# vwxyzjn/cleanrl

Measured on NVIDIA H100. Metric: env steps/sec (SPS) PPO Breakout num_envs=1024, higher is better.
Workload: dtype bf16

## Files before the change

cleanrl_b200/csrc/net_tc.cu:

```cuda
#include <cuda.h>
#include <algorithm>
#include "tc_base.cuh"
#include "tc_conv_win.cuh"
#include "tc_conv1_u8.cuh"
#include "tc_gemm_tma.cuh"
#include "tc_wgrad_win.cuh"
#include "tc_reduce.cuh"
#include "tc_aux.cuh"
#include "tc_heads.cuh"
#include "tc_heads_wide.cuh"
#include "tc_lstm.cuh"

namespace b200rl {

struct NatureLayout {
    int A;
    int64_t c1w, c1b, c2w, c2b, c3w, c3b, fcw, fcb, hw, hb, total;
    int64_t w1f, w2f, w2dg, w3f, w3dg, wfcf, wfcdg, w1l, w1sc, packed_total;
    bool wide; int G; int64_t whf, whdg, hbp;
    int64_t wih, whh, bih, bhh, whhp;
    explicit NatureLayout(int A_) : A(A_), wih(-1), whh(-1), bih(-1), bhh(-1), whhp(-1) {
        int64_t o = 0;
        c1w = o; o += 32 * 4 * 8 * 8;  c1b = o; o += 32;
        c2w = o; o += 64 * 32 * 4 * 4; c2b = o; o += 64;
        c3w = o; o += 64 * 64 * 3 * 3; c3b = o; o += 64;
        fcw = o; o += 512 * 3136;      fcb = o; o += 512;
        hw = o;  o += (int64_t)(A + 1) * 512;
        hb = o;  o += A + 1;
        total = o;
        int64_t q = 0;
        w1f = q; q += 32 * 256;
        w2f = q; q += 64 * 512;
        w2dg = q; q += 4 * 32 * 256;
        w3f = q; q += 64 * 576;
        w3dg = q; q += 64 * 576;
        wfcf = q; q += 512 * 3136;
        wfcdg = q; q += 3136 * 512;
        w1l = q; q += 64 * 256 / 2;
        w1sc = q; q += 64 * 2;
        wide = A + 1 > kMaxHeads;
        G = wide ? (int)ceil_div(A + 1, kWideHeadPad) * kWideHeadPad : 0;
        whf = whdg = hbp = 0;
        if (wide) {
            whf = q; q += (int64_t)G * 512;
            whdg = q; q += (int64_t)G * 512;
            hbp = q; q += (int64_t)G * 2;
        }
        packed_total = q;
    }
    struct Lstm {};
    NatureLayout(int A_, Lstm) : A(A_) {
        int64_t o = 0;
        c1w = o; o += 32 * 8 * 8;      c1b = o; o += 32;
        c2w = o; o += 64 * 32 * 4 * 4; c2b = o; o += 64;
        c3w = o; o += 64 * 64 * 3 * 3; c3b = o; o += 64;
        fcw = o; o += 512 * 3136;      fcb = o; o += 512;
// ... 9 lines not shown
        w3f = q; q += 64 * 576;
        w3dg = q; q += 64 * 576;
        wfcf = q; q += 512 * 3136;
        wfcdg = q; q += 3136 * 512;
        w1l = w1sc = -1;
        wide = true; G = 512;
        whf = q; q += 512 * 512;
        whdg = q; q += 512 * 512;
        hbp = q; q += 512 * 2;
        whhp = q; q += 512 * 128;
        packed_total = q;
    }
};

struct NatureActs {
    int64_t x0, act1, act2, act3, hid, dhid, dact3a, dact3b, dact2a, dact2b, dact1, m1, m2, m3, m4, total;
    explicit NatureActs(int64_t n, bool with_x0 = true) {
        int64_t o = 0;
        x0 = o; if (with_x0) o += n * 28224;
        act1 = o; o += n * 12800;
        act2 = o; o += n * 5184;
        act3 = o; o += n * 3136;
        hid = o;  o += n * 512;
        dhid = o; o += n * 512;
        dact3a = o; o += n * 5184;
        dact3b = o; o += n * 7744;
        dact2a = o; o += n * 6400;
        dact2b = o; o += n * 7744;
        dact1 = o; o += n * 14112;
        auto pad8 = [](int64_t v) { return (v + 7) & ~int64_t(7); };
        m1 = o; o += pad8(n * 100 * 4 * 2);
        m2 = o; o += pad8(n * 81 * 2 * 2);
        m3 = o; o += pad8(n * 49 * 2 * 2);
        m4 = o; o += pad8(n * 16 * 2);
        total = o;
    }
};

static void gemm_rowmajor(KGemmParams& p, const bf16* x, int64_t n, int nchunks) {
    memset(&p, 0, sizeof(p));
    p.scale = 1.f;
    p.A = x; p.M = n; p.nchunks = nchunks;
}


static void win_defaults(WinParams& p) { memset(&p, 0, sizeof(p)); p.scale = 1.f; }
static int round8(int v) { return (v + 7) & ~7; }
static void win_conv1(WinParams& p, const bf16* x0, const int64_t* rows, int64_t n) {
    p.A = x0; p.rows = rows; p.n = (int)n; p.G = 441; p.Wp = 21; p.M = n * 441;
    p.tpi_shift = 2;
    p.n_images = rows ? (int64_t)1 << 24 : n;
    p.ntaps = 4; p.shift[0] = 0; p.shift[1] = 1; p.shift[2] = 21; p.shift[3] = 22; p.WR = round8(128 + 22);
}
static void win_conv2(WinParams& p, const bf16* act1, int64_t n) {
    p.A = act1; p.n = (int)n; p.G = 100; p.Wp = 10; p.M = n * 100;
    p.ntaps = 4; p.shift[0] = 0; p.shift[1] = 1; p.shift[2] = 10; p.shift[3] = 11; p.WR = round8(128 + 11);
}
static void win_conv3(WinParams& p, const bf16* act2, int64_t n) {
    p.A = act2; p.n = (int)n; p.G = 81; p.Wp = 9; p.M = n * 81;
    p.ntaps = 9; for (int ky = 0; ky < 3; ++ky) for (int kx = 0; kx < 3; ++kx) p.shift[ky * 3 + kx] = ky * 9 + kx;
    p.WR = round8(128 + 20);
}
static void wgw_defaults(WGradWinParams& w) { memset(&w, 0, sizeof(w)); }

static const int kC1Ctas = 264, kC2Ctas = 132, kC3Ctas = 132;
static WPlan conv1_wgrad_plan(int64_t n, bool u8) {
    return u8 ? wgrad_plan(n * 512, kC2Ctas, 512) : wgrad_plan(n * 512, kC1Ctas, 128);
}
static WPlan conv2_wgrad_plan(int64_t n) { return wgrad_plan(n * 100, kC2Ctas, 128); }
static WPlan conv3_wgrad_plan(int64_t n) { return wgrad_plan(n * 81, kC3Ctas, 128); }

static size_t wgrad_win_bytes(int splits, int nslots) { return (size_t)splits * nslots * 64 * 64 * sizeof(float); }
static size_t wgrad_win_bias_bytes(int splits) { return (size_t)splits * 64 * sizeof(float); }
static int launch_wgrad_win(const WGradWinParams& p, int ctas, cudaStream_t s, const char* what) {
    const size_t smem = (size_t)kWgradWinStages * ((size_t)p.WRX * 128 * p.cpr + 128 * 128) + 4096 + 1024;
    static SmemAttrCache attr;
    if (int rc0 = attr.ensure(tc_wgrad_win, smem, what)) return rc0;
    CUtensorMap tmX, tmY;
    memset(&tmX, 0, sizeof(tmX)); memset(&tmY, 0, sizeof(tmY));
    const int use_tma = p.tpi_shift ? 0 : 1;
    if (p.rows_per_cta % 128 != 0) return fail(B200RL_ERR_INVALID_ARGUMENT, "%s: rows per CTA must be a multiple of 128", what);
    if (ctas < 1 || (int64_t)(ctas - 1) * p.rows_per_cta >= p.M)
        return fail(B200RL_ERR_INVALID_ARGUMENT, "%s: every row split must own at least one row", what);
    int rc;
    if (use_tma) {
        if (p.rows || p.ldy != 64 || p.ncolsY != 64)
            return fail(B200RL_ERR_INVALID_ARGUMENT, "%s: linear-grid mode needs contiguous rows and 64-channel dY", what);
        if ((rc = make_tmap_2d(&tmX, p.X, p.M, (int64_t)p.cpr * 64, p.WRX, what))) return rc;
        if ((rc = make_tmap_2d(&tmY, p.Y, p.M, 64, 128, what))) return rc;
    } else {
        if ((128 << p.tpi_shift) < p.G) return fail(B200RL_ERR_INVALID_ARGUMENT, "%s: steps per image too small", what);
        if ((rc = make_tmap_3d(&tmX, p.X, p.n_images, p.G, (int64_t)p.cpr * 64, p.WRX, what))) return rc;
    }
    const dim3 grid((unsigned)ceil_div(p.nslots / 2, kWgradWinTilesPerCta), ctas);
    tc_wgrad_win<<<grid, kWgradWinThreads, smem, s>>>(tmX, tmY, p, use_tma);
    return check_launch(what);
}

}

using namespace b200rl;

namespace b200rl {
static bool head_ok(int A) { return A >= 1 && A < kMaxWideHeads; }
static size_t wide_dhead_bytes(int64_t n, const NatureLayout& L) { return ((size_t)n * L.G * 2 + 255) & ~(size_t)255; }
static size_t wide_small_bytes(int64_t n, const NatureLayout& L, int A1) {
    return wide_dhead_bytes(n, L) + colsum_f32_ws(n, A1);
}

static int trunk_fwd(const NatureLayout& L, const NatureActs& Q, const float* params, const bf16* P, bf16* act, int64_t n,
                     cudaStream_t s) {
    int rc;
    KGemmParams p;
    WinParams wp;
    win_defaults(wp); win_conv2(wp, act + Q.act1, n);
    wp.Bw = P + L.w2f; wp.N = 64; wp.vH = 9; wp.vW = 9; wp.out_mode = WOUT_DENSE; wp.out = act + Q.act2;
    wp.bias = params + L.c2b; wp.relu = 1; wp.mask_out = reinterpret_cast<uint32_t*>(act + Q.m2);
    { ProfScope ps(s, "conv2_fwd", 2.0 * n * 81 * 64 * 512, (double)n * ((12800 + 5184) * 2 + 648));
      if (n <= 8192) { if ((rc = launch_conv_win_t<64, 2, 6, 4>(wp, s, "naturecnn/conv2"))) return rc; }
      else if ((rc = launch_conv_win_t<128, 2, 2, 4>(wp, s, "naturecnn/conv2"))) return rc; }
    win_defaults(wp); win_conv3(wp, act + Q.act2, n);
    wp.Bw = P + L.w3f; wp.N = 64; wp.vH = 7; wp.vW = 7; wp.out_mode = WOUT_DENSE; wp.out = act + Q.act3;
    wp.bias = params + L.c3b; wp.relu = 1; wp.mask_out = reinterpret_cast<uint32_t*>(act + Q.m3);
    { ProfScope ps(s, "conv3_fwd", 2.0 * n * 49 * 64 * 576, (double)n * ((5184 + 3136) * 2 + 392));
      if (n <= 8192) { if ((rc = launch_conv_win_t<64, 1, 8, 9>(wp, s, "naturecnn/conv3"))) return rc; }
      else if ((rc = launch_conv_win_t<128, 1, 4, 9>(wp, s, "naturecnn/conv3"))) return rc; }
    gemm_rowmajor(p, act + Q.act3, n, 49);
    p.Bw = P + L.wfcf; p.N = 512; p.out = act + Q.hid; p.ldo = 512; p.bias = params + L.fcb; p.relu = 1;
    p.mask_out = reinterpret_cast<uint32_t*>(act + Q.m4);
    { ProfScope ps(s, "fc_fwd", 2.0 * n * 512 * 3136, (double)n * (3136 + 512) * 2 + 512.0 * 3136 * 2);
      if (n <= 8192) { if ((rc = launch_gemm_tma<64, 6>(p, s, "naturecnn/fc"))) return rc; }
      else if ((rc = launch_gemm_tma<128, 3>(p, s, "naturecnn/fc"))) return rc; }
    return B200RL_OK;
}

static int trunk_bwd(const NatureLayout& L, const NatureActs& Q, const bf16* P, bf16* act, float* grads, int64_t n,
                     float* wsbig, float* wssmall, void* tail_ready_event, bool dact1_fused, cudaStream_t s) {
    int rc;
    KGemmParams p;
    {
        int splits;
        { ProfScope ps(s, "fc_wgrad", 2.0 * n * 512 * 3136, (double)n * (3136 + 512) * 2 + 512.0 * 3136 * 4);
          if ((splits = launch_wgrad_tma(act + Q.dhid, 512, act + Q.act3, 3136, n, wsbig, s, "naturecnn/fc_wgrad")) < 0) return splits; }
        { ProfScope ps(s, "wgrad_fold_bias", 0, 0);
          note_launches(1); tc_fold_fc<<<(unsigned)ceil_div((int64_t)512 * 3136, 256), 256, 0, s>>>(wsbig, splits, 512, 13 * 256, 512, 3136, 64, 49, 1.f, grads + L.fcw);
          if ((rc = colsum(act + Q.dhid, n, 512, 512, wssmall, grads + L.fcb, s))) return rc; }
        if (tail_ready_event) {
            cudaError_t e = cudaEventRecord(reinterpret_cast<cudaEvent_t>(tail_ready_event), s);
            if (e != cudaSuccess) return fail(B200RL_ERR_CUDA, "naturecnn_backward: cudaEventRecord: %s", cudaGetErrorString(e));
        }
        gemm_rowmajor(p, act + Q.dhid, n, 8);
        p.Bw = P + L.wfcdg; p.N = 3136; p.out = act + Q.dact3a; p.out2 = act + Q.dact3b; p.dual_dact3 = 1;
        p.ldo = 3136; p.mask_bits = reinterpret_cast<const uint32_t*>(act + Q.m3);
        { ProfScope ps(s, "fc_dgrad", 2.0 * n * 512 * 3136, (double)n * ((3136 + 512) * 2 + 392) + 512.0 * 3136 * 2);
          if ((rc = launch_gemm_tma<128, 3>(p, s, "naturecnn/fc_dgrad"))) return rc; }
    }
    WGradWinParams gw;
    WinParams wp;
    FoldWin fw;
    {
        wgw_defaults(gw);
        gw.X = act + Q.act2; gw.M = n * 81; gw.n = (int)n; gw.G = 81; gw.cpr = 1; gw.nslots = 10; gw.WRX = round8(128 + 20);
        for (int t = 0; t < 9; ++t) gw.shift[t] = (t / 3) * 9 + (t % 3);
        const int st[10] = {0, 1, 2, 3, 4, 5, 6, 7, 7, 8};
        for (int k = 0; k < 10; ++k) { gw.slot_tap[k] = st[k]; gw.slot_cc[k] = 0; }
        gw.Y = act + Q.dact3a; gw.ldy = 64; gw.ncolsY = 64;
        const WPlan pl = conv3_wgrad_plan(n);
        gw.rows_per_cta = pl.rows_per_cta; gw.ws = wsbig; gw.wsb = wssmall;
        { ProfScope ps(s, "conv3_wgrad", 2.0 * n * 49 * 64 * 576, (double)n * (5184 + 5184) * 2);
          if ((rc = launch_wgrad_win(gw, pl.splits, s, "naturecnn/conv3_wgrad"))) return rc; }
        memset(&fw, 0, sizeof(fw));
        fw.layer = 3; fw.S = pl.splits; fw.nslots = 10; fw.Cout = 64; fw.scale = 1.f; fw.bscale = 1.f;
        for (int k = 0; k < 10; ++k) { fw.slot_tap[k] = st[k]; fw.slot_skip[k] = (k == 8); }
        { ProfScope ps(s, "wgrad_fold_bias", 0, 0);
          fw.wsb = wssmall; fw.db = grads + L.c3b;
          tc_fold_win<<<(unsigned)ceil_div(640 * 64 + 64, 32), 256, 0, s>>>(wsbig, fw, grads + L.c3w);
          if ((rc = check_launch("naturecnn/conv3_fold"))) return rc; }
        win_defaults(wp);
        wp.A = act + Q.dact3b; wp.n = (int)n; wp.G = 121; wp.Wp = 11; wp.M = n * 121; wp.ntaps = 9;
// ... 462 lines not shown
```

cleanrl_b200/csrc/tc_conv_win.cuh:

```cuda
#pragma once
#include "tc_base.cuh"

namespace b200rl {
using namespace tc;

enum { WOUT_DENSE = 0, WOUT_S2D2 = 1, WOUT_DACT2 = 2, WOUT_DACT1 = 3 };
struct WinParams {
    const bf16* A;
    const int64_t* rows;
    int64_t M;
    int n, G, Wp;
    int tpi_shift;
    int64_t n_images;
    int ntaps;
    int shift[16];
    int WR;
    const bf16* Bw;
    int N;
    int vH, vW;
    int out_mode;
    bf16* out;
    bf16* out2;
    const uint32_t* mask_bits;
    uint32_t* mask_out;
// ... 219 lines not shown
}

template <int BN, int CPR, int STAGES, int NTAPS>
static int launch_conv_win(const WinParams& p, cudaStream_t s, const char* what) {
    if (p.ntaps != NTAPS) return fail(B200RL_ERR_INVALID_ARGUMENT, "%s: %d taps, kernel instance has %d", what, p.ntaps, NTAPS);
    if (p.out_mode != WOUT_S2D2 && p.out_mode != WOUT_DACT1)
        return fail(B200RL_ERR_INVALID_ARGUMENT, "%s: dense and conv3 data-gradient outputs run on tc_conv_win_t", what);
    if (p.out_mode == WOUT_DACT1 && (BN != 128 || p.N != 128))
        return fail(B200RL_ERR_INVALID_ARGUMENT, "%s: the conv2 data gradient stores 4 groups of 32 channels per cell", what);
    const size_t smem = (size_t)p.ntaps * CPR * BN * 128 + (size_t)STAGES * p.WR * 128 * CPR + conv_win_acc_bytes<BN>() + 1024;
    static SmemAttrCache attr;
    if (int rc = attr.ensure(tc_conv_win<BN, CPR, STAGES, NTAPS>, smem, what)) return rc;
    if ((int64_t)p.G * p.Wp >= 65536 || p.G < 1 || p.N % 32 != 0)
        return fail(B200RL_ERR_INVALID_ARGUMENT, "%s: grid %d x width %d outside the epilogue's multiply-shift range, or N %% 32 != 0", what, p.G, p.Wp);
    if (p.rows && !p.tpi_shift) return fail(B200RL_ERR_INVALID_ARGUMENT, "%s: the image gather needs image-aligned tiling", what);
    if (p.tpi_shift && (128 << p.tpi_shift) < p.G) return fail(B200RL_ERR_INVALID_ARGUMENT, "%s: tiles per image too small", what);
    const int total = p.tpi_shift ? (int)((int64_t)p.n << p.tpi_shift) : (int)ceil_div(p.M, 128);
    int grid = num_sms();
    if (grid > total) grid = total;
    CUtensorMap tmA, tmW;
    memset(&tmA, 0, sizeof(tmA));
    memset(&tmW, 0, sizeof(tmW));
    int rc;
    if (p.tpi_shift) rc = make_tmap_3d(&tmA, p.A, p.n_images, p.G, (int64_t)CPR * 64, p.WR, what);
    else rc = make_tmap_2d(&tmA, p.A, p.M, (int64_t)CPR * 64, p.WR, what);
    if (rc) return rc;
    if ((rc = make_tmap_2d(&tmW, p.Bw, p.N, (int64_t)NTAPS * CPR * 64, BN, what))) return rc;
    tc_conv_win<BN, CPR, STAGES, NTAPS><<<grid, kConvWinThreads, smem, s>>>(tmA, tmW, p, total);
    return check_launch(what);
}

constexpr int kConvWinTThreads = 384;
constexpr int kConvWinTLds = 64 + 4;
template <int BP>
__host__ __device__ constexpr size_t conv_win_t_stage_bytes() { return (size_t)2 * BP * kConvWinTLds * sizeof(float); }

template <int R>
__device__ __forceinline__ void stage_acc_transposed(float* st, int wg_tid, const float (&d)[R]) {
    const int co = ((wg_tid >> 5) << 4) + ((wg_tid & 31) >> 2), pos = (wg_tid & 3) * 2;
#pragma unroll
    for (int j = 0; j < R / 4; ++j) {
        float* p0 = st + (8 * j + pos) * kConvWinTLds + co;
        p0[0] = d[4 * j];
        p0[kConvWinTLds] = d[4 * j + 1];
        p0[8] = d[4 * j + 2];
        p0[kConvWinTLds + 8] = d[4 * j + 3];
    }
}

template <int BP, int CPR, int STAGES, int NTAPS>
__global__ void __launch_bounds__(kConvWinTThreads, 1) tc_conv_win_t(const __grid_constant__ CUtensorMap tmA,
                                                                     const __grid_constant__ CUtensorMap tmW, const WinParams p,
                                                                     int total_tiles) {
    static_assert(BP == 64 || BP % 128 == 0, "the epilogue's 128 threads per warpgroup cover whole position rows");
    static_assert(STAGES % 2 == 0, "each consumer warpgroup owns every other stage");
    constexpr int TPP = BP >= 128 ? 1 : 2;
    constexpr int PPR = 128 / TPP;
    constexpr int RPT = BP >= 128 ? BP / 128 : 1;
    constexpr int A_CHUNK = 64 * 128;
    constexpr int LDS = kConvWinTLds;
    extern __shared__ uint8_t smem_raw[];
    __shared__ uint64_t full_bar[STAGES], empty_bar[STAGES], w_bar;
    uint8_t* smem = smem_raw + ((1024u - (smem_u32(smem_raw) & 1023u)) & 1023u);
    const int tid = threadIdx.x, warp = tid >> 5;
    const int nchunks = NTAPS * CPR;
    const int IMG = p.WR * 128;
    const int STAGE_BYTES = IMG * CPR;
    uint8_t* sW = smem;
    uint8_t* sRing = smem + (size_t)nchunks * A_CHUNK;
    float* sAcc = reinterpret_cast<float*>(sRing + (size_t)STAGES * STAGE_BYTES);

    if (tid == 0) {
        for (int s = 0; s < STAGES; ++s) { mbar_init(&full_bar[s], 1); mbar_init(&empty_bar[s], 4); }
        mbar_init(&w_bar, 1);
        fence_barrier_init();
        tma_prefetch_desc(&tmA);
        tma_prefetch_desc(&tmW);
    }
    __syncthreads();
    const int tile_begin = (int)(((int64_t)total_tiles * blockIdx.x) / gridDim.x);
    const int tile_end = (int)(((int64_t)total_tiles * (blockIdx.x + 1)) / gridDim.x);

    if (warp == 0) {
        if (tid == 0) {
            uint32_t q = 0;
            for (int tile = tile_begin; tile < tile_end; ++tile, ++q) {
                const uint32_t s = q % STAGES;
                if (q >= (uint32_t)STAGES) mbar_wait(&empty_bar[s], ((q / STAGES) - 1) & 1);
                const uint32_t dst = smem_u32(sRing + (size_t)s * STAGE_BYTES);
                mbar_arrive_expect_tx(&full_bar[s], (uint32_t)STAGE_BYTES);
#pragma unroll
                for (int c = 0; c < CPR; ++c) tma_load_2d(dst + c * IMG, &tmA, c * 64, tile * BP, &full_bar[s]);
                if (q == 0) {
                    mbar_arrive_expect_tx(&w_bar, (uint32_t)(nchunks * A_CHUNK));
                    for (int j = 0; j < nchunks; ++j) tma_load_2d(smem_u32(sW + (size_t)j * A_CHUNK), &tmW, j * 64, 0, &w_bar);
                }
            }
        }
    } else if (warp >= 4) {
        const int wg = (warp - 4) >> 2, wt = tid & 127;
        float* st = sAcc + wg * BP * LDS;
        const uint32_t w_base = smem_u32(sW);
        const uint32_t mW = (65536u + (uint32_t)p.Wp - 1u) / (uint32_t)p.Wp;
        constexpr int NW = 2;
        const int pw = wt % PPR, gq = wt / PPR;
        float d[BP / 2];
#pragma unroll
        for (int e = 0; e < BP / 2; ++e) d[e] = 0.f;
        if (tile_begin + wg < tile_end) mbar_wait(&w_bar, 0);
        for (int tile = tile_begin + wg; tile < tile_end; tile += 2) {
            const uint32_t q = (uint32_t)(tile - tile_begin), s = q % STAGES;
            mbar_wait(&full_bar[s], (q / STAGES) & 1);
            wgmma_fence();
            const uint32_t win = smem_u32(sRing + (size_t)s * STAGE_BYTES);
#pragma unroll
            for (int t = 0; t < NTAPS; ++t) {
#pragma unroll
                for (int c = 0; c < CPR; ++c) {
                    const uint64_t b = desc_kmajor(win + (uint32_t)(c * IMG) + (uint32_t)p.shift[t] * 128u);
                    const uint64_t a = desc_kmajor(w_base + (uint32_t)((t * CPR + c) * A_CHUNK));
#pragma unroll
                    for (int kk = 0; kk < 4; ++kk)
                        WgmmaBf16<BP, 0, 0>::mma(d, a + 2 * kk, b + 2 * kk, (t | c | kk) != 0 ? 1u : 0u);
                }
            }
            wgmma_commit();
            bool valid[RPT];
            int64_t o1[RPT], o2[RPT], ob[RPT];
            uint32_t mb[RPT][NW];
#pragma unroll
            for (int rr = 0; rr < RPT; ++rr) {
                const int64_t r = (int64_t)tile * BP + rr * PPR + pw;
                const int i = (int)(r / p.G);
                const int rem = (int)(r - (int64_t)i * p.G);
                const int Y = (int)(((uint32_t)rem * mW) >> 16), X = rem - Y * p.Wp;
                valid[rr] = r < p.M && (Y < p.vH) && (X < p.vW);
                o2[rr] = 0;
                if (p.out_mode == WOUT_DENSE) {
                    const int64_t orow = ((int64_t)i * p.vH + Y) * p.vW + X;
                    o1[rr] = orow * p.N; ob[rr] = orow * (p.N >> 5);
                } else {
                    o1[rr] = ((int64_t)i * 100 + Y * 10 + X) * 64;
                    o2[rr] = ((int64_t)i * 121 + (Y + 1) * 11 + (X + 1)) * 64;
                    ob[rr] = ((int64_t)i * 81 + Y * 9 + X) * 2;
                }
                mb[rr][0] = mb[rr][1] = 0xFFFFFFFFu;
                if (p.mask_bits != nullptr && valid[rr]) {
                    const uint2 t = __ldg(reinterpret_cast<const uint2*>(p.mask_bits + ob[rr]));
                    mb[rr][0] = t.x; mb[rr][1] = t.y;
                }
            }
            wgmma_wait<0>();
            wgmma_fence_operands(d);
            if ((tid & 31) == 0) mbar_arrive(&empty_bar[s]);
            named_bar(1 + wg, 128);
            stage_acc_transposed(st, wt, d);
            named_bar(1 + wg, 128);
#pragma unroll
            for (int rr = 0; rr < RPT; ++rr) {
                float* srow = st + (rr * PPR + pw) * LDS;
#pragma unroll
                for (int g = 0; g < NW; ++g) {
                    if (TPP == 2 && g != gq) continue;
                    if (TPP == 1 && (!valid[rr] || g * 32 >= p.N)) continue;
                    uint32_t v[32];
#pragma unroll
                    for (int e = 0; e < 8; ++e) {
                        const float4 f = *reinterpret_cast<const float4*>(srow + g * 32 + 4 * e);
                        v[4 * e] = __float_as_uint(f.x); v[4 * e + 1] = __float_as_uint(f.y);
                        v[4 * e + 2] = __float_as_uint(f.z); v[4 * e + 3] = __float_as_uint(f.w);
                    }
                    if (TPP == 2) {
                        named_bar(1 + wg, 128);
                        if (!valid[rr] || g * 32 >= p.N) continue;
                    }
                    if (p.bias) {
                        const float4* bp = reinterpret_cast<const float4*>(p.bias + g * 32);
#pragma unroll
                        for (int e = 0; e < 8; ++e) {
                            const float4 bv = __ldg(bp + e);
                            v[4 * e] = __float_as_uint(fmaf(__uint_as_float(v[4 * e]), p.scale, bv.x));
                            v[4 * e + 1] = __float_as_uint(fmaf(__uint_as_float(v[4 * e + 1]), p.scale, bv.y));
                            v[4 * e + 2] = __float_as_uint(fmaf(__uint_as_float(v[4 * e + 2]), p.scale, bv.z));
                            v[4 * e + 3] = __float_as_uint(fmaf(__uint_as_float(v[4 * e + 3]), p.scale, bv.w));
                        }
                    } else {
#pragma unroll
                        for (int e = 0; e < 32; ++e) v[e] = __float_as_uint(__uint_as_float(v[e]) * p.scale);
                    }
                    if (p.relu) {
                        uint32_t bits = 0u;
#pragma unroll
                        for (int e = 0; e < 32; ++e) bits |= (__uint_as_float(v[e]) > 0.f ? 1u : 0u) << e;
                        if (p.mask_out) p.mask_out[ob[rr] + g] = bits;
                    }
                    if (p.mask_bits) {
#pragma unroll
                        for (int e = 0; e < 32; ++e) if (!((mb[rr][g] >> e) & 1u)) v[e] = 0u;
                    }
                    int4 w[4];
                    if (p.relu) {
#pragma unroll
                        for (int e = 0; e < 4; ++e) {
                            w[e].x = (int)pack_bf16x2_relu(__uint_as_float(v[8 * e]), __uint_as_float(v[8 * e + 1]));
                            w[e].y = (int)pack_bf16x2_relu(__uint_as_float(v[8 * e + 2]), __uint_as_float(v[8 * e + 3]));
                            w[e].z = (int)pack_bf16x2_relu(__uint_as_float(v[8 * e + 4]), __uint_as_float(v[8 * e + 5]));
                            w[e].w = (int)pack_bf16x2_relu(__uint_as_float(v[8 * e + 6]), __uint_as_float(v[8 * e + 7]));
                        }
                    } else {
#pragma unroll
                        for (int e = 0; e < 4; ++e) {
                            w[e].x = (int)pack_bf16x2(__uint_as_float(v[8 * e]), __uint_as_float(v[8 * e + 1]));
                            w[e].y = (int)pack_bf16x2(__uint_as_float(v[8 * e + 2]), __uint_as_float(v[8 * e + 3]));
                            w[e].z = (int)pack_bf16x2(__uint_as_float(v[8 * e + 4]), __uint_as_float(v[8 * e + 5]));
                            w[e].w = (int)pack_bf16x2(__uint_as_float(v[8 * e + 6]), __uint_as_float(v[8 * e + 7]));
                        }
                    }
                    int4* brow = reinterpret_cast<int4*>(srow) + 4 * g;
#pragma unroll
                    for (int e = 0; e < 4; ++e) brow[e] = w[e];
                }
                if (gq == 0) *reinterpret_cast<longlong2*>(srow + 64) = make_longlong2(valid[rr] ? o1[rr] : -1, o2[rr]);
            }
            named_bar(1 + wg, 128);
#pragma unroll
            for (int m = 0; m < BP / 16; ++m) {
                const int k = m * 128 + wt, part = k & 7;
                const float* srow = st + (k >> 3) * LDS;
                const longlong2 off = *reinterpret_cast<const longlong2*>(srow + 64);
                if (off.x < 0) continue;
                const int4 val = reinterpret_cast<const int4*>(srow)[part];
                *reinterpret_cast<int4*>(p.out + off.x + part * 8) = val;
                if (p.out_mode == WOUT_DACT2) *reinterpret_cast<int4*>(p.out2 + off.y + part * 8) = val;
            }
        }
    }
}

template <int BP, int CPR, int STAGES, int NTAPS>
static int launch_conv_win_t(WinParams p, cudaStream_t s, const char* what) {
    if (p.ntaps != NTAPS) return fail(B200RL_ERR_INVALID_ARGUMENT, "%s: %d taps, kernel instance has %d", what, p.ntaps, NTAPS);
    if (p.N != 64) return fail(B200RL_ERR_INVALID_ARGUMENT, "%s: N = %d, the kernel computes 64 output channels", what, p.N);
    if ((int64_t)p.G * p.Wp >= 65536 || p.G < 1)
        return fail(B200RL_ERR_INVALID_ARGUMENT, "%s: grid %d x width %d outside the epilogue's multiply-shift range", what, p.G, p.Wp);
    if (p.rows || p.tpi_shift) return fail(B200RL_ERR_INVALID_ARGUMENT, "%s: the channel-major kernel walks a contiguous linear grid", what);
    if (p.out_mode != WOUT_DENSE && p.out_mode != WOUT_DACT2)
        return fail(B200RL_ERR_INVALID_ARGUMENT, "%s: only bf16 dense and conv3 data-gradient outputs in this kernel", what);
    int maxs = 0;
    for (int t = 0; t < NTAPS; ++t) maxs = p.shift[t] > maxs ? p.shift[t] : maxs;
    p.WR = (BP + maxs + 7) & ~7;
    if (p.WR > 256) return fail(B200RL_ERR_INVALID_ARGUMENT, "%s: window of %d rows exceeds a TMA box", what, p.WR);
    const size_t smem = (size_t)NTAPS * CPR * 64 * 128 + (size_t)STAGES * p.WR * 128 * CPR + conv_win_t_stage_bytes<BP>() + 1024;
    static SmemAttrCache attr;
    if (int rc = attr.ensure(tc_conv_win_t<BP, CPR, STAGES, NTAPS>, smem, what)) return rc;
    const int total = (int)ceil_div(p.M, BP);
    int grid = num_sms();
    if (grid > total) grid = total;
    CUtensorMap tmA, tmW;
    memset(&tmA, 0, sizeof(tmA));
    memset(&tmW, 0, sizeof(tmW));
    if (int rc = make_tmap_2d(&tmA, p.A, p.M, (int64_t)CPR * 64, p.WR, what)) return rc;
    if (int rc = make_tmap_2d(&tmW, p.Bw, 64, (int64_t)NTAPS * CPR * 64, 64, what)) return rc;
    tc_conv_win_t<BP, CPR, STAGES, NTAPS><<<grid, kConvWinTThreads, smem, s>>>(tmA, tmW, p, total);
    return check_launch(what);
}

}
```

cleanrl_b200/csrc/tc_wgmma.cuh:

```cuda
#pragma once
#include <cstdint>

namespace b200rl { namespace tc {

__device__ __forceinline__ void wgmma_fence() { asm volatile("wgmma.fence.sync.aligned;" ::: "memory"); }
__device__ __forceinline__ void wgmma_commit() { asm volatile("wgmma.commit_group.sync.aligned;" ::: "memory"); }
template <int N>
__device__ __forceinline__ void wgmma_wait() { asm volatile("wgmma.wait_group.sync.aligned %0;" ::"n"(N) : "memory"); }
template <class T, int R>
__device__ __forceinline__ void wgmma_fence_operands(T (&d)[R]) {
#pragma unroll
    for (int i = 0; i < R; ++i) asm volatile("" : "+r"(reinterpret_cast<uint32_t&>(d[i]))::"memory");
}

template <int N, int TA, int TB> struct WgmmaBf16;
template <int TA, int TB> struct WgmmaBf16<32, TA, TB> {
    __device__ __forceinline__ static void mma(float (&d)[16], uint64_t adesc, uint64_t bdesc, uint32_t accumulate) {
        asm volatile(
            "{\n\t.reg .pred p;\n\tsetp.ne.b32 p, %18, 0;\n\t"
            "wgmma.mma_async.sync.aligned.m64n32k16.f32.bf16.bf16 {"
            "%0, %1, %2, %3, %4, %5, %6, %7, %8, %9, %10, %11, %12, %13, %14, %15"
            "}, %16, %17, p, 1, 1, %19, %20;\n\t}\n"
            : "+f"(d[0]), "+f"(d[1]), "+f"(d[2]), "+f"(d[3]), "+f"(d[4]), "+f"(d[5]), "+f"(d[6]), "+f"(d[7]),
              "+f"(d[8]), "+f"(d[9]), "+f"(d[10]), "+f"(d[11]), "+f"(d[12]), "+f"(d[13]), "+f"(d[14]), "+f"(d[15])
            : "l"(adesc), "l"(bdesc), "r"(accumulate), "n"(TA), "n"(TB));
    }
};
template <int TA, int TB> struct WgmmaBf16<64, TA, TB> {
    __device__ __forceinline__ static void mma(float (&d)[32], uint64_t adesc, uint64_t bdesc, uint32_t accumulate) {
        asm volatile(
            "{\n\t.reg .pred p;\n\tsetp.ne.b32 p, %34, 0;\n\t"
            "wgmma.mma_async.sync.aligned.m64n64k16.f32.bf16.bf16 {"
            "%0, %1, %2, %3, %4, %5, %6, %7, %8, %9, %10, %11, %12, %13, %14, %15, "
            "%16, %17, %18, %19, %20, %21, %22, %23, %24, %25, %26, %27, %28, %29, %30, %31"
            "}, %32, %33, p, 1, 1, %35, %36;\n\t}\n"
            : "+f"(d[0]), "+f"(d[1]), "+f"(d[2]), "+f"(d[3]), "+f"(d[4]), "+f"(d[5]), "+f"(d[6]), "+f"(d[7]),
              "+f"(d[8]), "+f"(d[9]), "+f"(d[10]), "+f"(d[11]), "+f"(d[12]), "+f"(d[13]), "+f"(d[14]), "+f"(d[15]),
              "+f"(d[16]), "+f"(d[17]), "+f"(d[18]), "+f"(d[19]), "+f"(d[20]), "+f"(d[21]), "+f"(d[22]), "+f"(d[23]),
              "+f"(d[24]), "+f"(d[25]), "+f"(d[26]), "+f"(d[27]), "+f"(d[28]), "+f"(d[29]), "+f"(d[30]), "+f"(d[31])
            : "l"(adesc), "l"(bdesc), "r"(accumulate), "n"(TA), "n"(TB));
    }
};
template <int TA, int TB> struct WgmmaBf16<128, TA, TB> {
    __device__ __forceinline__ static void mma(float (&d)[64], uint64_t adesc, uint64_t bdesc, uint32_t accumulate) {
        asm volatile(
            "{\n\t.reg .pred p;\n\tsetp.ne.b32 p, %66, 0;\n\t"
            "wgmma.mma_async.sync.aligned.m64n128k16.f32.bf16.bf16 {"
            "%0, %1, %2, %3, %4, %5, %6, %7, %8, %9, %10, %11, %12, %13, %14, %15, "
            "%16, %17, %18, %19, %20, %21, %22, %23, %24, %25, %26, %27, %28, %29, %30, %31, "
            "%32, %33, %34, %35, %36, %37, %38, %39, %40, %41, %42, %43, %44, %45, %46, %47, "
            "%48, %49, %50, %51, %52, %53, %54, %55, %56, %57, %58, %59, %60, %61, %62, %63"
            "}, %64, %65, p, 1, 1, %67, %68;\n\t}\n"
            : "+f"(d[0]), "+f"(d[1]), "+f"(d[2]), "+f"(d[3]), "+f"(d[4]), "+f"(d[5]), "+f"(d[6]), "+f"(d[7]),
              "+f"(d[8]), "+f"(d[9]), "+f"(d[10]), "+f"(d[11]), "+f"(d[12]), "+f"(d[13]), "+f"(d[14]), "+f"(d[15]),
              "+f"(d[16]), "+f"(d[17]), "+f"(d[18]), "+f"(d[19]), "+f"(d[20]), "+f"(d[21]), "+f"(d[22]), "+f"(d[23]),
              "+f"(d[24]), "+f"(d[25]), "+f"(d[26]), "+f"(d[27]), "+f"(d[28]), "+f"(d[29]), "+f"(d[30]), "+f"(d[31]),
              "+f"(d[32]), "+f"(d[33]), "+f"(d[34]), "+f"(d[35]), "+f"(d[36]), "+f"(d[37]), "+f"(d[38]), "+f"(d[39]),
              "+f"(d[40]), "+f"(d[41]), "+f"(d[42]), "+f"(d[43]), "+f"(d[44]), "+f"(d[45]), "+f"(d[46]), "+f"(d[47]),
              "+f"(d[48]), "+f"(d[49]), "+f"(d[50]), "+f"(d[51]), "+f"(d[52]), "+f"(d[53]), "+f"(d[54]), "+f"(d[55]),
              "+f"(d[56]), "+f"(d[57]), "+f"(d[58]), "+f"(d[59]), "+f"(d[60]), "+f"(d[61]), "+f"(d[62]), "+f"(d[63])
            : "l"(adesc), "l"(bdesc), "r"(accumulate), "n"(TA), "n"(TB));
    }
};
template <int TA, int TB> struct WgmmaBf16<256, TA, TB> {
    __device__ __forceinline__ static void mma(float (&d)[128], uint64_t adesc, uint64_t bdesc, uint32_t accumulate) {
        asm volatile(
            "{\n\t.reg .pred p;\n\tsetp.ne.b32 p, %130, 0;\n\t"
            "wgmma.mma_async.sync.aligned.m64n256k16.f32.bf16.bf16 {"
            "%0, %1, %2, %3, %4, %5, %6, %7, %8, %9, %10, %11, %12, %13, %14, %15, "
            "%16, %17, %18, %19, %20, %21, %22, %23, %24, %25, %26, %27, %28, %29, %30, %31, "
            "%32, %33, %34, %35, %36, %37, %38, %39, %40, %41, %42, %43, %44, %45, %46, %47, "
            "%48, %49, %50, %51, %52, %53, %54, %55, %56, %57, %58, %59, %60, %61, %62, %63, "
            "%64, %65, %66, %67, %68, %69, %70, %71, %72, %73, %74, %75, %76, %77, %78, %79, "
            "%80, %81, %82, %83, %84, %85, %86, %87, %88, %89, %90, %91, %92, %93, %94, %95, "
            "%96, %97, %98, %99, %100, %101, %102, %103, %104, %105, %106, %107, %108, %109, %110, %111, "
            "%112, %113, %114, %115, %116, %117, %118, %119, %120, %121, %122, %123, %124, %125, %126, %127"
            "}, %128, %129, p, 1, 1, %131, %132;\n\t}\n"
            : "+f"(d[0]), "+f"(d[1]), "+f"(d[2]), "+f"(d[3]), "+f"(d[4]), "+f"(d[5]), "+f"(d[6]), "+f"(d[7]),
              "+f"(d[8]), "+f"(d[9]), "+f"(d[10]), "+f"(d[11]), "+f"(d[12]), "+f"(d[13]), "+f"(d[14]), "+f"(d[15]),
              "+f"(d[16]), "+f"(d[17]), "+f"(d[18]), "+f"(d[19]), "+f"(d[20]), "+f"(d[21]), "+f"(d[22]), "+f"(d[23]),
              "+f"(d[24]), "+f"(d[25]), "+f"(d[26]), "+f"(d[27]), "+f"(d[28]), "+f"(d[29]), "+f"(d[30]), "+f"(d[31]),
              "+f"(d[32]), "+f"(d[33]), "+f"(d[34]), "+f"(d[35]), "+f"(d[36]), "+f"(d[37]), "+f"(d[38]), "+f"(d[39]),
              "+f"(d[40]), "+f"(d[41]), "+f"(d[42]), "+f"(d[43]), "+f"(d[44]), "+f"(d[45]), "+f"(d[46]), "+f"(d[47]),
              "+f"(d[48]), "+f"(d[49]), "+f"(d[50]), "+f"(d[51]), "+f"(d[52]), "+f"(d[53]), "+f"(d[54]), "+f"(d[55]),
              "+f"(d[56]), "+f"(d[57]), "+f"(d[58]), "+f"(d[59]), "+f"(d[60]), "+f"(d[61]), "+f"(d[62]), "+f"(d[63]),
              "+f"(d[64]), "+f"(d[65]), "+f"(d[66]), "+f"(d[67]), "+f"(d[68]), "+f"(d[69]), "+f"(d[70]), "+f"(d[71]),
              "+f"(d[72]), "+f"(d[73]), "+f"(d[74]), "+f"(d[75]), "+f"(d[76]), "+f"(d[77]), "+f"(d[78]), "+f"(d[79]),
              "+f"(d[80]), "+f"(d[81]), "+f"(d[82]), "+f"(d[83]), "+f"(d[84]), "+f"(d[85]), "+f"(d[86]), "+f"(d[87]),
              "+f"(d[88]), "+f"(d[89]), "+f"(d[90]), "+f"(d[91]), "+f"(d[92]), "+f"(d[93]), "+f"(d[94]), "+f"(d[95]),
              "+f"(d[96]), "+f"(d[97]), "+f"(d[98]), "+f"(d[99]), "+f"(d[100]), "+f"(d[101]), "+f"(d[102]), "+f"(d[103]),
              "+f"(d[104]), "+f"(d[105]), "+f"(d[106]), "+f"(d[107]), "+f"(d[108]), "+f"(d[109]), "+f"(d[110]), "+f"(d[111]),
              "+f"(d[112]), "+f"(d[113]), "+f"(d[114]), "+f"(d[115]), "+f"(d[116]), "+f"(d[117]), "+f"(d[118]), "+f"(d[119]),
// ... 35 lines not shown
```

Baseline: 1.281 million.

## Fuse conv2 and conv3 forward into one persistent per-image kernel

Replaces the separate conv2 and conv3 windowed-conv launches with one persistent kernel that processes a whole image per warpgroup. conv2 output is built in shared memory (bias, ReLU, mask bits) and fed straight into conv3's wgmma, while act2 is still written to global memory for backward. This removes one launch and the global round trip of act2 between the two convs. The cost is a fixed per-image schedule with more synchronisation, padded 96-column conv2 tiles, and a single CTA per SM. The now-unused BP=64 path in the old window-conv kernel is removed.

After: 1.330 million, median of 6. 1.04x the previous value.

```diff
diff --git a/cleanrl_b200/csrc/net_tc.cu b/cleanrl_b200/csrc/net_tc.cu
--- a/cleanrl_b200/csrc/net_tc.cu
+++ b/cleanrl_b200/csrc/net_tc.cu
@@ -2,6 +2,7 @@
 #include <algorithm>
 #include "tc_base.cuh"
 #include "tc_conv_win.cuh"
+#include "tc_conv23.cuh"
 #include "tc_conv1_u8.cuh"
 #include "tc_gemm_tma.cuh"
 #include "tc_wgrad_win.cuh"
@@ -117,15 +118,6 @@
     p.n_images = rows ? (int64_t)1 << 24 : n;
     p.ntaps = 4; p.shift[0] = 0; p.shift[1] = 1; p.shift[2] = 21; p.shift[3] = 22; p.WR = round8(128 + 22);
 }
-static void win_conv2(WinParams& p, const bf16* act1, int64_t n) {
-    p.A = act1; p.n = (int)n; p.G = 100; p.Wp = 10; p.M = n * 100;
-    p.ntaps = 4; p.shift[0] = 0; p.shift[1] = 1; p.shift[2] = 10; p.shift[3] = 11; p.WR = round8(128 + 11);
-}
-static void win_conv3(WinParams& p, const bf16* act2, int64_t n) {
-    p.A = act2; p.n = (int)n; p.G = 81; p.Wp = 9; p.M = n * 81;
-    p.ntaps = 9; for (int ky = 0; ky < 3; ++ky) for (int kx = 0; kx < 3; ++kx) p.shift[ky * 3 + kx] = ky * 9 + kx;
-    p.WR = round8(128 + 20);
-}
 static void wgw_defaults(WGradWinParams& w) { memset(&w, 0, sizeof(w)); }
 
 static const int kC1Ctas = 264, kC2Ctas = 132, kC3Ctas = 132;
@@ -177,19 +169,12 @@
                      cudaStream_t s) {
     int rc;
     KGemmParams p;
-    WinParams wp;
-    win_defaults(wp); win_conv2(wp, act + Q.act1, n);
-    wp.Bw = P + L.w2f; wp.N = 64; wp.vH = 9; wp.vW = 9; wp.out_mode = WOUT_DENSE; wp.out = act + Q.act2;
-    wp.bias = params + L.c2b; wp.relu = 1; wp.mask_out = reinterpret_cast<uint32_t*>(act + Q.m2);
-    { ProfScope ps(s, "conv2_fwd", 2.0 * n * 81 * 64 * 512, (double)n * ((12800 + 5184) * 2 + 648));
-      if (n <= 8192) { if ((rc = launch_conv_win_t<64, 2, 6, 4>(wp, s, "naturecnn/conv2"))) return rc; }
-      else if ((rc = launch_conv_win_t<128, 2, 2, 4>(wp, s, "naturecnn/conv2"))) return rc; }
-    win_defaults(wp); win_conv3(wp, act + Q.act2, n);
-    wp.Bw = P + L.w3f; wp.N = 64; wp.vH = 7; wp.vW = 7; wp.out_mode = WOUT_DENSE; wp.out = act + Q.act3;
-    wp.bias = params + L.c3b; wp.relu = 1; wp.mask_out = reinterpret_cast<uint32_t*>(act + Q.m3);
-    { ProfScope ps(s, "conv3_fwd", 2.0 * n * 49 * 64 * 576, (double)n * ((5184 + 3136) * 2 + 392));
-      if (n <= 8192) { if ((rc = launch_conv_win_t<64, 1, 8, 9>(wp, s, "naturecnn/conv3"))) return rc; }
-      else if ((rc = launch_conv_win_t<128, 1, 4, 9>(wp, s, "naturecnn/conv3"))) return rc; }
+    Conv23Params cp;
+    cp.n = (int)n; cp.b2 = params + L.c2b; cp.b3 = params + L.c3b; cp.act2 = act + Q.act2; cp.act3 = act + Q.act3;
+    cp.m2 = reinterpret_cast<uint32_t*>(act + Q.m2); cp.m3 = reinterpret_cast<uint32_t*>(act + Q.m3);
+    { ProfScope ps(s, "conv23_fwd", 2.0 * n * 81 * 64 * 512 + 2.0 * n * 49 * 64 * 576,
+                   (double)n * (12800 * 2 + 5184 * 2 + 648 + 3136 * 2 + 392));
+      if ((rc = launch_conv23_fwd(act + Q.act1, P + L.w2f, P + L.w3f, cp, s, "naturecnn/conv23"))) return rc; }
     gemm_rowmajor(p, act + Q.act3, n, 49);
     p.Bw = P + L.wfcf; p.N = 512; p.out = act + Q.hid; p.ldo = 512; p.bias = params + L.fcb; p.relu = 1;
     p.mask_out = reinterpret_cast<uint32_t*>(act + Q.m4);
diff --git a/cleanrl_b200/csrc/tc_conv23.cuh b/cleanrl_b200/csrc/tc_conv23.cuh
--- /dev/null
+++ b/cleanrl_b200/csrc/tc_conv23.cuh
@@ -0,0 +1,218 @@
+#pragma once
+#include "tc_conv_win.cuh"
+
+namespace b200rl {
+using namespace tc;
+
+struct Conv23Params {
+    int n;
+    const float* b2;
+    const float* b3;
+    bf16* act2;
+    bf16* act3;
+    uint32_t* m2;
+    uint32_t* m3;
+};
+
+constexpr int kConv23Threads = 384;
+constexpr int kC23WinRows = 112;
+constexpr int kC23Chunk = 64 * 128;
+constexpr int kC23StageBytes = 2 * kC23WinRows * 128;
+constexpr int kC23ImgBytes = 64 * 64 * 4;
+constexpr size_t kC23Smem = (size_t)(8 + 9) * kC23Chunk + 2 * kC23StageBytes + 2 * kC23ImgBytes + 1024;
+static_assert(96 * kConvWinTLds * 4 <= kC23StageBytes, "conv2's fp32 staging fits its window stage");
+static_assert(88 * 128 <= kC23ImgBytes, "the act2 image and its zero tail fit the conv3 staging");
+
+__device__ __forceinline__ uint32_t conv23_group(const float* srow, int g, int sw, const float* bias, int4 (&w)[4]) {
+    float v[32];
+    const float4* bp = reinterpret_cast<const float4*>(bias + g * 32);
+#pragma unroll
+    for (int e = 0; e < 8; ++e) {
+        const float4 f = reinterpret_cast<const float4*>(srow)[(8 * g + e) ^ sw];
+        const float4 bv = __ldg(bp + e);
+        v[4 * e] = fmaf(f.x, 1.f, bv.x); v[4 * e + 1] = fmaf(f.y, 1.f, bv.y);
+        v[4 * e + 2] = fmaf(f.z, 1.f, bv.z); v[4 * e + 3] = fmaf(f.w, 1.f, bv.w);
+    }
+    uint32_t bits = 0u;
+#pragma unroll
+    for (int e = 0; e < 32; ++e) bits |= (v[e] > 0.f ? 1u : 0u) << e;
+#pragma unroll
+    for (int e = 0; e < 4; ++e) {
+        w[e].x = (int)pack_bf16x2_relu(v[8 * e], v[8 * e + 1]);
+        w[e].y = (int)pack_bf16x2_relu(v[8 * e + 2], v[8 * e + 3]);
+        w[e].z = (int)pack_bf16x2_relu(v[8 * e + 4], v[8 * e + 5]);
+        w[e].w = (int)pack_bf16x2_relu(v[8 * e + 6], v[8 * e + 7]);
+    }
+    return bits;
+}
+
+__device__ __forceinline__ void stage_acc_transposed_sw(float* st, int wg_tid, const float (&d)[32]) {
+    const int co = ((wg_tid >> 5) << 4) + ((wg_tid & 31) >> 2), pos = (wg_tid & 3) * 2;
+#pragma unroll
+    for (int j = 0; j < 8; ++j) {
+        const int r0 = 8 * j + pos, r1 = r0 + 1;
+        st[r0 * 64 + (co ^ ((r0 & 7) << 2))] = d[4 * j];
+        st[r1 * 64 + (co ^ ((r1 & 7) << 2))] = d[4 * j + 1];
+        st[r0 * 64 + ((co + 8) ^ ((r0 & 7) << 2))] = d[4 * j + 2];
+        st[r1 * 64 + ((co + 8) ^ ((r1 & 7) << 2))] = d[4 * j + 3];
+    }
+}
+
+__global__ void __launch_bounds__(kConv23Threads, 1) tc_conv23_fwd(const __grid_constant__ CUtensorMap tmA,
+                                                                   const __grid_constant__ CUtensorMap tmW2,
+                                                                   const __grid_constant__ CUtensorMap tmW3, const Conv23Params p) {
+    constexpr int IMG = kC23WinRows * 128;
+    constexpr int LDS = kConvWinTLds;
+    extern __shared__ uint8_t smem_raw[];
+    __shared__ uint64_t full_bar[2], empty_bar[2], w2_bar, w3_bar;
+    uint8_t* smem = smem_raw + ((1024u - (smem_u32(smem_raw) & 1023u)) & 1023u);
+    const int tid = threadIdx.x, warp = tid >> 5;
+    uint8_t* sW2 = smem;
+    uint8_t* sW3 = sW2 + 8 * kC23Chunk;
+    uint8_t* sRing = sW3 + 9 * kC23Chunk;
+    uint8_t* sImg = sRing + 2 * kC23StageBytes;
+
+    if (tid == 0) {
+        for (int s = 0; s < 2; ++s) { mbar_init(&full_bar[s], 1); mbar_init(&empty_bar[s], 4); }
+        mbar_init(&w2_bar, 1);
+        mbar_init(&w3_bar, 1);
+        fence_barrier_init();
+        tma_prefetch_desc(&tmA);
+        tma_prefetch_desc(&tmW2);
+        tma_prefetch_desc(&tmW3);
+    }
+    __syncthreads();
+    const int img_begin = (int)(((int64_t)p.n * blockIdx.x) / gridDim.x);
+    const int img_end = (int)(((int64_t)p.n * (blockIdx.x + 1)) / gridDim.x);
+
+    if (warp == 0) {
+        if (tid == 0) {
+            bool w3_sent = false;
+            uint32_t q = 0;
+            for (int img = img_begin; img < img_end; ++img, ++q) {
+                const uint32_t s = q & 1;
+                if (q >= 2) mbar_wait(&empty_bar[s], ((q >> 1) - 1) & 1);
+                const uint32_t dst = smem_u32(sRing + (size_t)s * kC23StageBytes);
+                mbar_arrive_expect_tx(&full_bar[s], (uint32_t)kC23StageBytes);
+                tma_load_3d(dst, &tmA, 0, 0, img, &full_bar[s]);
+                tma_load_3d(dst + IMG, &tmA, 64, 0, img, &full_bar[s]);
+                if (q == 0) {
+                    mbar_arrive_expect_tx(&w2_bar, (uint32_t)(8 * kC23Chunk));
+                    for (int j = 0; j < 8; ++j) tma_load_2d(smem_u32(sW2 + (size_t)j * kC23Chunk), &tmW2, j * 64, 0, &w2_bar);
+                }
+                if (!w3_sent && (q == 1 || img + 1 == img_end)) {
+                    mbar_arrive_expect_tx(&w3_bar, (uint32_t)(9 * kC23Chunk));
+                    for (int j = 0; j < 9; ++j) tma_load_2d(smem_u32(sW3 + (size_t)j * kC23Chunk), &tmW3, j * 64, 0, &w3_bar);
+                    w3_sent = true;
+                }
+            }
+        }
+    } else if (warp >= 4) {
+        const int wg = (warp - 4) >> 2, wt = tid & 127;
+        uint8_t* img2 = sImg + (size_t)wg * kC23ImgBytes;
+        float* st3 = reinterpret_cast<float*>(img2);
+        const uint32_t w2_base = smem_u32(sW2), w3_base = smem_u32(sW3), img2_base = smem_u32(img2);
+        const int shift2[4] = {0, 1, 10, 11};
+        float d2[48], d3[32];
+#pragma unroll
+        for (int e = 0; e < 48; ++e) d2[e] = 0.f;
+#pragma unroll
+        for (int e = 0; e < 32; ++e) d3[e] = 0.f;
+        if (img_begin + wg < img_end) mbar_wait(&w2_bar, 0);
+        for (int img = img_begin + wg; img < img_end; img += 2) {
+            const uint32_t q = (uint32_t)(img - img_begin), s = q & 1;
+            const int64_t i = img;
+            mbar_wait(&full_bar[s], (q >> 1) & 1);
+            wgmma_fence();
+            uint8_t* stage = sRing + (size_t)s * kC23StageBytes;
+            const uint32_t win = smem_u32(stage);
+#pragma unroll
+            for (int t = 0; t < 4; ++t) {
+#pragma unroll
+                for (int c = 0; c < 2; ++c) {
+                    const uint64_t b = desc_kmajor(win + (uint32_t)(c * IMG) + (uint32_t)shift2[t] * 128u);
+                    const uint64_t a = desc_kmajor(w2_base + (uint32_t)((t * 2 + c) * kC23Chunk));
+#pragma unroll
+                    for (int kk = 0; kk < 4; ++kk) WgmmaBf16<96, 0, 0>::mma(d2, a + 2 * kk, b + 2 * kk, (t | c | kk) != 0 ? 1u : 0u);
+                }
+            }
+            wgmma_commit();
+            wgmma_wait<0>();
+            wgmma_fence_operands(d2);
+            float* st2 = reinterpret_cast<float*>(stage);
+            stage_acc_transposed(st2, wt, d2);
+            named_bar(1 + wg, 128);
+#pragma unroll
+            for (int pass = 0; pass < 2; ++pass) {
+                const int k = pass * 128 + wt;
+                if (k >= 192) continue;
+                const int pos = k % 96, g = k / 96;
+                const int Y = pos / 10, X = pos - 10 * Y;
+                if (Y >= 9 || X >= 9) continue;
+                const int r = Y * 9 + X;
+                int4 w[4];
+                p.m2[(i * 81 + r) * 2 + g] = conv23_group(st2 + pos * LDS, g, 0, p.b2, w);
+#pragma unroll
+                for (int e = 0; e < 4; ++e) *reinterpret_cast<int4*>(img2 + img_off(r, 4 * g + e)) = w[e];
+            }
+            if (wt < 56) *reinterpret_cast<int4*>(img2 + 81 * 128 + wt * 16) = make_int4(0, 0, 0, 0);
+            fence_proxy_async_smem();
+            named_bar(1 + wg, 128);
+            if ((tid & 31) == 0) mbar_arrive(&empty_bar[s]);
+            if (q < 2) mbar_wait(&w3_bar, 0);
+            wgmma_fence();
+#pragma unroll
+            for (int t = 0; t < 9; ++t) {
+                const uint64_t b = desc_kmajor(img2_base + (uint32_t)((t / 3) * 9 + t % 3) * 128u);
+                const uint64_t a = desc_kmajor(w3_base + (uint32_t)(t * kC23Chunk));
+#pragma unroll
+                for (int kk = 0; kk < 4; ++kk) WgmmaBf16<64, 0, 0>::mma(d3, a + 2 * kk, b + 2 * kk, (t | kk) != 0 ? 1u : 0u);
+            }
+            wgmma_commit();
+            int4* a2 = reinterpret_cast<int4*>(p.act2 + i * 5184);
+#pragma unroll
+            for (int m = 0; m < 6; ++m) {
+                const int k = m * 128 + wt;
+                if (k < 648) a2[k] = *reinterpret_cast<const int4*>(img2 + img_off(k >> 3, k & 7));
+            }
+            wgmma_wait<0>();
+            wgmma_fence_operands(d3);
+            named_bar(1 + wg, 128);
+            stage_acc_transposed_sw(st3, wt, d3);
+            named_bar(1 + wg, 128);
+            {
+                const int pw = wt & 63, g = wt >> 6;
+                const int y = pw / 9, x = pw - 9 * y;
+                if (y < 7 && x < 7) {
+                    const int64_t orow = i * 49 + y * 7 + x;
+                    int4 w[4];
+                    p.m3[orow * 2 + g] = conv23_group(st3 + pw * 64, g, pw & 7, p.b3, w);
+                    bf16* dst = p.act3 + orow * 64 + g * 32;
+                    st_global_32b(dst, w[0], w[1]);
+                    st_global_32b(dst + 16, w[2], w[3]);
+                }
+            }
+        }
+    }
+}
+
+static int launch_conv23_fwd(const bf16* act1, const bf16* w2, const bf16* w3, const Conv23Params& p, cudaStream_t s,
+                             const char* what) {
+    if (p.n < 1) return fail(B200RL_ERR_INVALID_ARGUMENT, "%s: n = %d", what, p.n);
+    static SmemAttrCache attr;
+    if (int rc = attr.ensure(tc_conv23_fwd, kC23Smem, what)) return rc;
+    int grid = num_sms();
+    if (grid > p.n) grid = p.n;
+    CUtensorMap tmA, tmW2, tmW3;
+    memset(&tmA, 0, sizeof(tmA));
+    memset(&tmW2, 0, sizeof(tmW2));
+    memset(&tmW3, 0, sizeof(tmW3));
+    int rc;
+    if ((rc = make_tmap_3d(&tmA, act1, p.n, 100, 128, kC23WinRows, what))) return rc;
+    if ((rc = make_tmap_2d(&tmW2, w2, 64, 512, 64, what))) return rc;
+    if ((rc = make_tmap_2d(&tmW3, w3, 64, 576, 64, what))) return rc;
+    tc_conv23_fwd<<<grid, kConv23Threads, kC23Smem, s>>>(tmA, tmW2, tmW3, p);
+    return check_launch(what);
+}
+
+}
diff --git a/cleanrl_b200/csrc/tc_conv_win.cuh b/cleanrl_b200/csrc/tc_conv_win.cuh
--- a/cleanrl_b200/csrc/tc_conv_win.cuh
+++ b/cleanrl_b200/csrc/tc_conv_win.cuh
@@ -295,11 +295,10 @@
 __global__ void __launch_bounds__(kConvWinTThreads, 1) tc_conv_win_t(const __grid_constant__ CUtensorMap tmA,
                                                                      const __grid_constant__ CUtensorMap tmW, const WinParams p,
                                                                      int total_tiles) {
-    static_assert(BP == 64 || BP % 128 == 0, "the epilogue's 128 threads per warpgroup cover whole position rows");
+    static_assert(BP % 128 == 0, "the epilogue's 128 threads per warpgroup cover whole position rows");
     static_assert(STAGES % 2 == 0, "each consumer warpgroup owns every other stage");
-    constexpr int TPP = BP >= 128 ? 1 : 2;
-    constexpr int PPR = 128 / TPP;
-    constexpr int RPT = BP >= 128 ? BP / 128 : 1;
+    constexpr int PPR = 128;
+    constexpr int RPT = BP / 128;
     constexpr int A_CHUNK = 64 * 128;
     constexpr int LDS = kConvWinTLds;
     extern __shared__ uint8_t smem_raw[];
@@ -346,7 +345,7 @@
         const uint32_t w_base = smem_u32(sW);
         const uint32_t mW = (65536u + (uint32_t)p.Wp - 1u) / (uint32_t)p.Wp;
         constexpr int NW = 2;
-        const int pw = wt % PPR, gq = wt / PPR;
+        const int pw = wt;
         float d[BP / 2];
 #pragma unroll
         for (int e = 0; e < BP / 2; ++e) d[e] = 0.f;
@@ -404,18 +403,13 @@
                 float* srow = st + (rr * PPR + pw) * LDS;
 #pragma unroll
                 for (int g = 0; g < NW; ++g) {
-                    if (TPP == 2 && g != gq) continue;
-                    if (TPP == 1 && (!valid[rr] || g * 32 >= p.N)) continue;
+                    if (!valid[rr] || g * 32 >= p.N) continue;
                     uint32_t v[32];
 #pragma unroll
                     for (int e = 0; e < 8; ++e) {
                         const float4 f = *reinterpret_cast<const float4*>(srow + g * 32 + 4 * e);
                         v[4 * e] = __float_as_uint(f.x); v[4 * e + 1] = __float_as_uint(f.y);
                         v[4 * e + 2] = __float_as_uint(f.z); v[4 * e + 3] = __float_as_uint(f.w);
-                    }
-                    if (TPP == 2) {
-                        named_bar(1 + wg, 128);
-                        if (!valid[rr] || g * 32 >= p.N) continue;
                     }
                     if (p.bias) {
                         const float4* bp = reinterpret_cast<const float4*>(p.bias + g * 32);
@@ -463,7 +457,7 @@
 #pragma unroll
                     for (int e = 0; e < 4; ++e) brow[e] = w[e];
                 }
-                if (gq == 0) *reinterpret_cast<longlong2*>(srow + 64) = make_longlong2(valid[rr] ? o1[rr] : -1, o2[rr]);
+                *reinterpret_cast<longlong2*>(srow + 64) = make_longlong2(valid[rr] ? o1[rr] : -1, o2[rr]);
             }
             named_bar(1 + wg, 128);
 #pragma unroll
diff --git a/cleanrl_b200/csrc/tc_wgmma.cuh b/cleanrl_b200/csrc/tc_wgmma.cuh
--- a/cleanrl_b200/csrc/tc_wgmma.cuh
+++ b/cleanrl_b200/csrc/tc_wgmma.cuh
@@ -38,6 +38,24 @@
               "+f"(d[8]), "+f"(d[9]), "+f"(d[10]), "+f"(d[11]), "+f"(d[12]), "+f"(d[13]), "+f"(d[14]), "+f"(d[15]),
               "+f"(d[16]), "+f"(d[17]), "+f"(d[18]), "+f"(d[19]), "+f"(d[20]), "+f"(d[21]), "+f"(d[22]), "+f"(d[23]),
               "+f"(d[24]), "+f"(d[25]), "+f"(d[26]), "+f"(d[27]), "+f"(d[28]), "+f"(d[29]), "+f"(d[30]), "+f"(d[31])
+            : "l"(adesc), "l"(bdesc), "r"(accumulate), "n"(TA), "n"(TB));
+    }
+};
+template <int TA, int TB> struct WgmmaBf16<96, TA, TB> {
+    __device__ __forceinline__ static void mma(float (&d)[48], uint64_t adesc, uint64_t bdesc, uint32_t accumulate) {
+        asm volatile(
+            "{\n\t.reg .pred p;\n\tsetp.ne.b32 p, %50, 0;\n\t"
+            "wgmma.mma_async.sync.aligned.m64n96k16.f32.bf16.bf16 {"
+            "%0, %1, %2, %3, %4, %5, %6, %7, %8, %9, %10, %11, %12, %13, %14, %15, "
+            "%16, %17, %18, %19, %20, %21, %22, %23, %24, %25, %26, %27, %28, %29, %30, %31, "
+            "%32, %33, %34, %35, %36, %37, %38, %39, %40, %41, %42, %43, %44, %45, %46, %47"
+            "}, %48, %49, p, 1, 1, %51, %52;\n\t}\n"
+            : "+f"(d[0]), "+f"(d[1]), "+f"(d[2]), "+f"(d[3]), "+f"(d[4]), "+f"(d[5]), "+f"(d[6]), "+f"(d[7]),
+              "+f"(d[8]), "+f"(d[9]), "+f"(d[10]), "+f"(d[11]), "+f"(d[12]), "+f"(d[13]), "+f"(d[14]), "+f"(d[15]),
+              "+f"(d[16]), "+f"(d[17]), "+f"(d[18]), "+f"(d[19]), "+f"(d[20]), "+f"(d[21]), "+f"(d[22]), "+f"(d[23]),
+              "+f"(d[24]), "+f"(d[25]), "+f"(d[26]), "+f"(d[27]), "+f"(d[28]), "+f"(d[29]), "+f"(d[30]), "+f"(d[31]),
+              "+f"(d[32]), "+f"(d[33]), "+f"(d[34]), "+f"(d[35]), "+f"(d[36]), "+f"(d[37]), "+f"(d[38]), "+f"(d[39]),
+              "+f"(d[40]), "+f"(d[41]), "+f"(d[42]), "+f"(d[43]), "+f"(d[44]), "+f"(d[45]), "+f"(d[46]), "+f"(d[47])
             : "l"(adesc), "l"(bdesc), "r"(accumulate), "n"(TA), "n"(TB));
     }
 };
```
